# Peilun-Tommy-Li/pHNN-MPC

Hardware: AMD Instinct MI355X
Metric: pHNN-MPC rollouts+grads/sec, cartpole H=50 batch=65536 (higher is better)
Workload: dtype f32

## Files before the change

### phnn_mpc_amd/csrc/phnn_kernels.hip.h

```cpp
#pragma once
#include <hip/hip_runtime.h>

#include <type_traits>

#include "../../include/phnn_mpc.h"
#include "phnn_riccati.hip.h"

#define DEV __device__ __forceinline__
#ifdef PHNN_CACHED_TAPE
#define PHNN_NT_STORE(v, p) (*(p) = (v))
#define PHNN_NT_LOAD(p) (*(p))
#else
#define PHNN_NT_STORE(v, p) __builtin_nontemporal_store((v), (p))
#define PHNN_NT_LOAD(p) __builtin_nontemporal_load((p))
#endif

using f32x4 = __attribute__((ext_vector_type(4))) float;
using f32x2 = __attribute__((ext_vector_type(2))) float;

constexpr int kTileB = 16;
#ifndef PHNN_KMAXWAVES
#define PHNN_KMAXWAVES 8
#endif
constexpr int kMaxWaves = PHNN_KMAXWAVES;
// ... 403 lines not shown
  static constexpr int PART = HID * RS * 2;
  static constexpr int FLOATS = 2 * PART / 4;
};

DEV f16x8 in_frag_h(f32x4 x) {
  f32x2 v01 = {x[0], x[1]}, v23 = {x[2], x[3]};
  f16x2 h01 = __builtin_convertvector(v01, f16x2), h23 = __builtin_convertvector(v23, f16x2);
  f32x2 r01 = residual_h(h01, v01), r23 = residual_h(h23, v23);
  u32x4 B = {__builtin_bit_cast(unsigned, h01), __builtin_bit_cast(unsigned, h23),
             __builtin_bit_cast(unsigned, __builtin_convertvector(r01, f16x2)),
             __builtin_bit_cast(unsigned, __builtin_convertvector(r23, f16x2))};
  return __builtin_bit_cast(f16x8, B);
}
constexpr int kInFragH(int T) { return T * 64 * 4; }
template <int T>
DEV void in_layer_h(Act<T>& o, const float* Wh, Lane ln, f16x8 xf) {
  keep_lds_reads_local();
#pragma unroll
  for (int nt = 0; nt < T; ++nt) o.v[nt] = mfma_h(*reinterpret_cast<const f16x8*>(Wh + (nt * 64 + ln.lane) * 4), xf, o.v[nt]);
}
constexpr int kInHFwd = 1, kInHRecomp = 2, kInHHvp = 4, kInHNet1 = 8, kInHNet1Adj = 16;
#ifndef PHNN_INH_MASK
#define PHNN_INH_MASK (kInHFwd | kInHRecomp | kInHHvp | kInHNet1 | kInHNet1Adj)
#endif
template <int T, int MM, int SITE>
DEV void in_layer_mm(Act<T>& o, const float* Lnet, int oF, int oFh, Lane ln, f32x4 x, int tile0 = 0) {
  if constexpr (MM == MM_F16X2 && (PHNN_INH_MASK & SITE) != 0) in_layer_h<T>(o, Lnet + oFh + tile0 * 256, ln, in_frag_h(x));
  else in_layer<T>(o, Lnet + oF + tile0 * 64, ln, sel4(x, ln.q));
}

DEV void mfma3x2(f32x4& o0, f32x4& o1, const f16x8 (&a)[2][2], f16x8 xh, f16x8 xl) {
  o0 = mfma_h(a[0][1], xh, o0);
  o1 = mfma_h(a[1][1], xh, o1);
  o0 = mfma_h(a[0][0], xl, o0);
  o1 = mfma_h(a[1][0], xl, o1);
  o0 = mfma_h(a[0][0], xh, o0);
  o1 = mfma_h(a[1][0], xh, o1);
}

struct NoEpi {
  DEV void operator()(int, int) const {}
};
#ifndef PHNN_FUSE_SITES
#define PHNN_FUSE_SITES 15
#endif
#ifdef PHNN_NO_FUSED_EPILOGUE
constexpr int kFuseSites = 0;
#else
constexpr int kFuseSites = PHNN_FUSE_SITES;
#endif
constexpr int kFuseK1Act = 1, kFuseK1Red = 2, kFuseK2Act = 4, kFuseK2Red = 8;
#define PHNN_FUSE_K1 (kFuseK1Act | kFuseK1Red)
#define PHNN_FUSE_K2 (kFuseK2Act | kFuseK2Red)
template <int T, class Epi>
DEV void epi_slices(Epi& epi, int P, int s) {
  constexpr int NS = T / 2;
#pragma unroll
  for (int j = (4 * s) / NS; j < (4 * (s + 1)) / NS; ++j) epi(P, j);
}
template <int T, class Epi>
DEV void epi_tail(Epi& epi) {
#pragma unroll
  for (int j = 0; j < 4; ++j) epi(T / 2 - 1, j);
}

template <int T, class Epi = NoEpi>
DEV void sq_fwd_h(Act<T>& o, const float* Wimg, Lane ln, const Split2<T>& in, Epi epi = Epi()) {
  constexpr bool FUSED = !std::is_same_v<Epi, NoEpi>;
  using I = HfImg<16 * T>;
  keep_lds_reads_local();
  matrix_phase_begin();
  const char* base = reinterpret_cast<const char*>(Wimg) + ln.i * (I::RS * 2) + ln.q * 16;
#ifndef PHNN_NO_PREFETCH_FRAGS
  {
    constexpr int PD = 1, NB = PD + 1;
    f16x8 a[NB][2][2];
    auto loadg = [&](int g, f16x8 (&dst)[2][2]) {
      const int n0 = 2 * (g / (T / 2)), s = g % (T / 2);
#pragma unroll
      for (int gg = 0; gg < 2; ++gg)
#pragma unroll
        for (int p = 0; p < 2; ++p)
          dst[gg][p] = *reinterpret_cast<const f16x8*>(base + p * I::PART + (n0 + gg) * 16 * (I::RS * 2) + s * 64);
    };
    constexpr int NG = (T / 2) * (T / 2);
#pragma unroll
    for (int g = 0; g < PD && g < NG; ++g) loadg(g, a[g % NB]);
#pragma unroll
    for (int g = 0; g < NG; ++g) {
      if (g + PD < NG) loadg(g + PD, a[(g + PD) % NB]);
      __builtin_amdgcn_sched_barrier(0);
      const int n0 = 2 * (g / (T / 2)), s = g % (T / 2);
      mfma3x2(o.v[n0], o.v[n0 + 1], a[g % NB], in.h[s], in.l[s]);
      if constexpr (FUSED)
        if (n0 > 0) epi_slices<T>(epi, n0 / 2 - 1, s);
      __builtin_amdgcn_sched_barrier(0);
    }
    matrix_phase_end();
    if constexpr (FUSED) epi_tail<T>(epi);
    return;
  }
#endif
#pragma unroll
  for (int n0 = 0; n0 < T; n0 += 2) {
    if constexpr (FUSED)
      if (n0 > 0) {
// ... 323 lines not shown
    a = z > 0.f ? z : expm1f(z);
    d1 = z > 0.f ? 1.0f : __builtin_amdgcn_exp2f(z * 1.4426950408889634f);
  } else if (ACT == ACT_GELU) {
    const float c = gelu_cdf(z);
    a = z * c;
    d1 = __builtin_fmaf(z, gelu_pdf(z), c);
  } else {
    const float s = __builtin_amdgcn_rcpf(1.0f + __builtin_amdgcn_exp2f(z * -1.4426950408889634f));
    a = z * s;
    d1 = __builtin_fmaf(a, 1.0f - s, s);
  }
}
template <int ACT>
DEV float act_d2(float z) {
  if (ACT == ACT_RELU) return 0.0f;
  if (ACT == ACT_ELU) return z > 0.f ? 0.0f : __builtin_amdgcn_exp2f(z * 1.4426950408889634f);
  if (ACT == ACT_GELU) return gelu_pdf(z) * fmaxf(__builtin_fmaf(-z, z, 2.0f), -3.0e38f);
  const float s = __builtin_amdgcn_rcpf(1.0f + __builtin_amdgcn_exp2f(z * -1.4426950408889634f));
  return s * (1.0f - s) * __builtin_fmaf(z, 1.0f - 2.0f * s, 2.0f);
}
template <int ACT, int T>
DEV void act_of(const Act<T>& z, Act<T>& a) {
#pragma unroll
  for (int t = 0; t < T; ++t)
#pragma unroll
    for (int r = 0; r < 4; ++r) {
      float av, d;
      act_eval<ACT>(z.v[t][r], av, d);
      a.v[t][r] = av;
    }
}
template <int ACT, int T>
DEV void mul_d1(Act<T>& g, const Act<T>& z) {
#pragma unroll
  for (int t = 0; t < T; ++t)
#pragma unroll
    for (int r = 0; r < 4; ++r) {
      float a, d;
      act_eval<ACT>(z.v[t][r], a, d);
      g.v[t][r] *= d;
    }
}

constexpr int TAPE_NONE = 0, TAPE_MPC = 1, TAPE_TRAIN = 2;
template <class M, int TK>
constexpr int tape_floats() {
  if constexpr (TK == TAPE_MPC && M::CURV) return M::TAPE_C;
  else return M::STASH;
}

template <int HID>
struct HTape {
  Act<HID / 16> a1, a2, q1;
};

template <int HID, bool WANT_H, int ACT>
DEV f32x4 hnet_grad_g(const float* L, Lane ln, f32x4 x, HTape<HID>& tp, float& Hval) {
  using Y = LayH2<HID, MM_F32>;
  constexpr int T = Y::T;
  load_vec<T>(tp.a1, L + Y::oB1, ln);
  in_layer<T>(tp.a1, L + Y::oW1f, ln, sel4(x, ln.q));
  {
    Act<T> a;
    act_of<ACT, T>(tp.a1, a);
    load_vec<T>(tp.a2, L + Y::oB2, ln);
    sq_fwd<T, T>(tp.a2, L + Y::oW2, ln, a);
  }
  Act<T> g;
  float s = 0.f;
  keep_lds_reads_local();
#pragma unroll
  for (int t = 0; t < T; ++t) {
    f32x4 w3 = *reinterpret_cast<const f32x4*>(L + Y::oW3 + 16 * t + 4 * ln.q);
#pragma unroll
    for (int r = 0; r < 4; ++r) {
      float a, d;
      act_eval<ACT>(tp.a2.v[t][r], a, d);
      if (WANT_H) s = __builtin_fmaf(w3[r], a, s);
      g.v[t][r] = w3[r] * d;
    }
  }
  if (WANT_H) Hval = reduce_q(s) + L[Y::oB3];
  zero_act<T>(tp.q1);
  sq_bwd<T, T>(tp.q1, L + Y::oW2, ln, g);
#pragma unroll
  for (int t = 0; t < T; ++t) g.v[t] = tp.q1.v[t];
  mul_d1<ACT, T>(g, tp.a1);
  return to4_rep<T>(L + Y::oW1T, ln, g);
}
template <int HID, int ACT>
DEV void hnet_layer1_g(const float* L, Lane ln, f32x4 x, Act<HID / 16>& z1) {
  using Y = LayH2<HID, MM_F32>;
  load_vec<Y::T>(z1, L + Y::oB1, ln);
  in_layer<Y::T>(z1, L + Y::oW1f, ln, sel4(x, ln.q));
}
template <int HID, int ACT>
DEV f32x4 hnet_hvp_g(const float* L, Lane ln, HTape<HID>& tp, f32x4 v) {
  using Y = LayH2<HID, MM_F32>;
  constexpr int T = Y::T;
  Act<T> ad1, w;
  zero_act<T>(ad1);
  in_layer<T>(ad1, L + Y::oW1f, ln, sel4(v, ln.q));
#pragma unroll
  for (int t = 0; t < T; ++t)
#pragma unroll
    for (int r = 0; r < 4; ++r) {
      const float z = tp.a1.v[t][r], zd = ad1.v[t][r];
// ... 58 lines not shown
        if (e == 2 && t + 1 < T) {
          if (WANT_H) w3 = *reinterpret_cast<const f32x4*>(L + Y::oW3 + 16 * (t + 1) + 4 * ln.q);
          w3b = *reinterpret_cast<const f32x4*>(L + Y::oW3B + 16 * (t + 1) + 4 * ln.q);
        }
        split_put_h<T>(spg, P, j, g);
      };
    };
    if (kPreScaled<T> && c == 1.0f) sq_fwd_h<T>(tp.a2, L + Y::oW2, ln, sp, act(std::true_type()));
    else sq_fwd_h<T>(tp.a2, L + Y::oW2, ln, sp, act(std::false_type()));
  } else if (MM == MM_BF16X3) {
    Split3<T> sp;
    split_act<T>(tp.a1, sp);
    sq_fwd_bf<T>(tp.a2, L + Y::oW2, ln, sp);
  } else if (MM == MM_F16X2) {
    Split2<T> sp;
    split_act_h<T>(tp.a1, sp);
    sq_fwd_h<T>(tp.a2, L + Y::oW2, ln, sp);
  } else {
    sq_fwd<T, T>(tp.a2, L + Y::oW2, ln, tp.a1);
  }
  if constexpr (FUSE_ACT) {
  } else if (MM == MM_F16X2 || kPreScaled<T>) {
    const float c = L[Y::oB3 + 1];
    if (kPreScaled<T> && c == 1.0f) {
      tanh_act_pre<T>(tp.a2);
    } else {
#pragma unroll
      for (int t = 0; t < T; ++t)
#pragma unroll
        for (int r = 0; r < 4; ++r) tp.a2.v[t][r] = tanh_scaled(tp.a2.v[t][r], c);
    }
  } else {
    tanh_act<T>(tp.a2);
  }
  Act<T> g;
  keep_lds_reads_local();
  if constexpr (!FUSE_ACT) {
#pragma unroll
    for (int t = 0; t < T; ++t) {
      if (WANT_H) {
        f32x4 w3 = *reinterpret_cast<const f32x4*>(L + Y::oW3 + 16 * t + 4 * ln.q);
#pragma unroll
        for (int r = 0; r < 4; ++r) s = __builtin_fmaf(w3[r], tp.a2.v[t][r], s);
      }
      f32x4 w3b = *reinterpret_cast<const f32x4*>(L + Y::oW3B + 16 * t + 4 * ln.q);
      g.v[t] = w3b * dtanh(tp.a2.v[t]);
    }
  }
  if (WANT_H) Hval = reduce_q(s) + L[Y::oB3];
  zero_act<T>(tp.q1);
  if constexpr (FUSABLE) {
    if constexpr (!FUSE_ACT) split_act_h<T>(g, spg);
    if constexpr (FUSE_RED) {
      To4Pairs<T> red(L + Y::oW1T, ln);
      sq_bwd_h<T>(tp.q1, L + Y::oW2, ln, spg, [&](int P, int j) {
        const int t = 2 * P + (j >> 1), e = 2 * (j & 1);
        const float a0 = tp.a1.v[t][e], a1 = tp.a1.v[t][e + 1];
        red.put(P, j, tp.q1.v[t][e] * __builtin_fmaf(-a0, a0, 1.0f), tp.q1.v[t][e + 1] * __builtin_fmaf(-a1, a1, 1.0f));
      });
      return red.finish();
    } else {
      sq_bwd_h<T>(tp.q1, L + Y::oW2, ln, spg);
    }
  } else if (MM == MM_BF16X3) {
    Split3<T> sp;
    split_act<T>(g, sp);
    sq_bwd_bf<T>(tp.q1, L + Y::oW2, ln, sp);
  } else if (MM == MM_F16X2) {
    Split2<T> sp;
    split_act_h<T>(g, sp);
    sq_bwd_h<T>(tp.q1, L + Y::oW2, ln, sp);
  } else {
    sq_bwd<T, T>(tp.q1, L + Y::oW2, ln, g);
  }
#pragma unroll
  for (int t = 0; t < T; ++t) g.v[t] = tp.q1.v[t] * dtanh(tp.a1.v[t]);
  return to4_rep<T>(L + Y::oW1T, ln, g);
}

template <int HID, int MM, int ACT = ACT_TANH>
DEV void hnet_layer1(const float* L, Lane ln, f32x4 z, Act<HID / 16>& a1) {
  if constexpr (ACT != ACT_TANH) return hnet_layer1_g<HID, ACT>(L, ln, z, a1);
  using Y = LayH2<HID, MM>;
  load_vec<Y::T>(a1, L + Y::oB1, ln);
  in_layer_mm<Y::T, MM, kInHRecomp>(a1, L, Y::oW1f, Y::oW1h, ln, z);
  tanh_act_pre<Y::T>(a1);
}

template <int HID>
struct CurvImg {
  static constexpr int RS = HID + 16, PART = 10 * RS * 2;
  static constexpr int oConst = 2 * PART / 4;
  static constexpr int FLOATS = oConst + 4;
};
struct Curv {
  float m[16];
};
template <int T>
DEV void hnet_curv_operand(const Act<T>& q1, const Act<T>& a1, Split2<T>& sp) {
  Act<T> c;
#pragma unroll
  for (int t = 0; t < T; ++t) c.v[t] = (q1.v[t] * dtanh(a1.v[t])) * a1.v[t];
  split_act_h<T>(c, sp);
}
template <int HID>
DEV f32x4 hnet_curv_kstep(const float* P, Lane ln, int s, f16x8 ch, f16x8 cl) {
  using I = CurvImg<HID>;
  keep_lds_reads_local();
  const int a = ln.i >> 2, b = ln.i & 3, lo = a < b ? a : b, hi = a < b ? b : a;
  const int row = (lo * (9 - lo)) / 2 + (hi - lo);
  const char* base = reinterpret_cast<const char*>(P) + row * (I::RS * 2) + ln.q * 16 + s * 64;
  const f16x8 ah = *reinterpret_cast<const f16x8*>(base);
  const f16x8 al = *reinterpret_cast<const f16x8*>(base + I::PART);
  return mfma_h(ah, ch, mfma_h(ah, cl, mfma_h(al, ch, splat4(0.f))));
}
template <int HID>
DEV f32x4 hnet_curv(const float* P, Lane ln, const HTape<HID>& tp) {
  constexpr int T = HID / 16;
  Split2<T> sp;
  hnet_curv_operand<T>(tp.q1, tp.a1, sp);
  f32x4 tot = hnet_curv_kstep<HID>(P, ln, 0, sp.h[0], sp.l[0]);
#pragma unroll
  for (int s = 1; s < T / 2; ++s) tot = tot + hnet_curv_kstep<HID>(P, ln, s, sp.h[s], sp.l[s]);
  return tot * P[CurvImg<HID>::oConst];
}
DEV void spread_curv(f32x4 mine, Lane ln, Curv& c) {
#pragma unroll
  for (int r = 0; r < 4; ++r)
#pragma unroll
    for (int j = 0; j < 4; ++j) c.m[4 * r + j] = __shfl(mine[j], 16 * r + ln.i);
}
DEV f32x4 curv_apply(const Curv& c, f32x4 v) {
  f32x4 o;
#pragma unroll
  for (int r = 0; r < 4; ++r) {
    float s = 0.f;
#pragma unroll
    for (int j = 0; j < 4; ++j) s = __builtin_fmaf(c.m[4 * r + j], v[j], s);
    o[r] = s;
  }
  return o;
}

template <int HID, bool COMPACT>
DEV void hnet_tape_store(float* stash, int oC, const float* P, Lane ln, const HTape<HID>& tp, f32x4 dH) {
  constexpr int T = HID / 16;
  store_act<T>(stash, ln, tp.a2);
  if constexpr (COMPACT) {
    if (ln.q == 0) PHNN_NT_STORE(dH, reinterpret_cast<f32x4*>(stash + T * 256) + ln.i);
    PHNN_NT_STORE(hnet_curv<HID>(P, ln, tp), reinterpret_cast<f32x4*>(stash + oC) + ln.i * 4 + ln.q);
  } else {
    store_act<T>(stash + T * 256, ln, tp.q1);
    if (ln.q == 0) PHNN_NT_STORE(dH, reinterpret_cast<f32x4*>(stash + 2 * T * 256) + ln.i);
  }
}
template <int T, bool COMPACT>
DEV f32x4 tape_load_dH(const float* stash, Lane ln) {
  return PHNN_NT_LOAD(reinterpret_cast<const f32x4*>(stash + (COMPACT ? 1 : 2) * T * 256) + ln.i);
}
DEV void load_curv(const float* src, Lane ln, Curv& c) {
  const f32x4* p = reinterpret_cast<const f32x4*>(src) + ln.i * 4;
#pragma unroll
  for (int k = 0; k < 4; ++k) {
    f32x4 v = PHNN_NT_LOAD(p + k);
#pragma unroll
    for (int e = 0; e < 4; ++e) c.m[4 * k + e] = v[e];
  }
}
template <int HID, bool COMPACT>
DEV void hnet_tape_load(const float* stash, int oC, Lane ln, HTape<HID>& tp, Curv& cv) {
  constexpr int T = HID / 16;
  load_act<T>(stash, ln, tp.a2);
  if constexpr (COMPACT) load_curv(stash + oC, ln, cv);
  else load_act<T>(stash + T * 256, ln, tp.q1);
}

DEV int pow2_exponent(float mx) {
  int e = 0;
  (void)__builtin_frexpf(mx, &e);
  return (mx > 0.f && mx < 3.0e38f) ? e : 0;
}
DEV f32x4 pow2_normalise(f32x4 v, float& unscale) {
  float mx = fmaxf(fmaxf(__builtin_fabsf(v[0]), __builtin_fabsf(v[1])), fmaxf(__builtin_fabsf(v[2]), __builtin_fabsf(v[3])));
  const int e = pow2_exponent(mx);
  v = v * __builtin_ldexpf(1.0f, -e);
  unscale = __builtin_ldexpf(1.0f, e);
  return v;
}

template <int HID, int MM = MM_F32, bool WG = false, int ACT = ACT_TANH, int SITE = kInHHvp, bool CQ = false, int FE = 0>
DEV f32x4 hnet_hvp(const float* L, Lane ln, HTape<HID>& tp, f32x4 v, float* rec = nullptr, const Curv* cv = nullptr) {
  static_assert(!CQ || (MM == MM_F16X2 && ACT == ACT_TANH && !WG), "the curvature block exists for f16x2 Tanh MPC kernels");
  if constexpr (ACT != ACT_TANH) {
    static_assert(!WG, "weight-gradient kernels exist for Tanh models only");
    return hnet_hvp_g<HID, ACT>(L, ln, tp, v);
  }
  using Y = LayH2<HID, MM>;
  constexpr int T = Y::T;
  float unscale = 1.0f;
  if (MM == MM_F16X2) v = pow2_normalise(v, unscale);
  Act<T> ad1, w;
  zero_act<T>(ad1);
  in_layer_mm<T, MM, SITE>(ad1, L, Y::oW1f, Y::oW1h, ln, v);
#pragma unroll
  for (int t = 0; t < T; ++t) ad1.v[t] = dtanh(tp.a1.v[t]) * ad1.v[t];
  if constexpr (!CQ) {
#pragma unroll
    for (int t = 0; t < T; ++t) tp.q1.v[t] = tp.q1.v[t] * (tp.a1.v[t] * ad1.v[t]);
  }
  zero_act<T>(w);
  constexpr bool FUSABLE = CQ && T >= 2 && T % 2 == 0;
  constexpr bool FUSE_ACT = FUSABLE && (FE & kFuseSites & kFuseK2Act) != 0, FUSE_RED = FUSABLE && (FE & kFuseSites & kFuseK2Red) != 0;
  Split2<T> spw{};
  if constexpr (FUSE_ACT) {
    Split2<T> sp;
    split_act_h<T>(ad1, sp);
    f32x4 w3 = *reinterpret_cast<const f32x4*>(L + Y::oW3S + 4 * ln.q);
    sq_fwd_h<T>(w, L + Y::oW2, ln, sp, [&](int P, int j) {
      const int t = 2 * P + (j >> 1), e = 2 * (j & 1);
      f32x2 x;
#pragma unroll
      for (int k = 0; k < 2; ++k) {
        const float a2 = tp.a2.v[t][e + k];
        const float ad2 = __builtin_fmaf(-a2, a2, 1.0f) * w.v[t][e + k];
        x[k] = w3[e + k] * (a2 * ad2);
      }
      if (e == 2 && t + 1 < T) w3 = *reinterpret_cast<const f32x4*>(L + Y::oW3S + 16 * (t + 1) + 4 * ln.q);
      split_put_h<T>(spw, P, j, x);
    });
  } else {
    if (MM == MM_BF16X3) {
      Split3<T> sp;
      split_act<T>(ad1, sp);
      sq_fwd_bf<T>(w, L + Y::oW2, ln, sp);
    } else if (MM == MM_F16X2) {
      Split2<T> sp;
      split_act_h<T>(ad1, sp);
      sq_fwd_h<T>(w, L + Y::oW2, ln, sp);
    } else {
      sq_fwd<T, T>(w, L + Y::oW2, ln, ad1);
    }
    keep_lds_reads_local();
#pragma unroll
    for (int t = 0; t < T; ++t) {
      f32x4 w3 = *reinterpret_cast<const f32x4*>(L + Y::oW3S + 16 * t + 4 * ln.q);
      f32x4 a2 = tp.a2.v[t];
      f32x4 ad2 = dtanh(a2) * w.v[t];
      if (WG) PHNN_REC_STORE(ad2 * unscale, reinterpret_cast<f32x4*>(rec + 2 * T * 256) + t * 64 + ln.lane);
      w.v[t] = w3 * (a2 * ad2);
    }
  }
  Act<T> qd;
  zero_act<T>(qd);
  if constexpr (FUSABLE) {
    if constexpr (!FUSE_ACT) split_act_h<T>(w, spw);
    if constexpr (FUSE_RED) {
      To4Pairs<T> red(L + Y::oW1T, ln);
      sq_bwd_h<T>(qd, L + Y::oW2, ln, spw, [&](int P, int j) {
        const int t = 2 * P + (j >> 1), e = 2 * (j & 1);
        const float a0 = tp.a1.v[t][e], a1 = tp.a1.v[t][e + 1];
        red.put(P, j, qd.v[t][e] * __builtin_fmaf(-a0, a0, 1.0f), qd.v[t][e + 1] * __builtin_fmaf(-a1, a1, 1.0f));
      });
      return (red.finish() * (-2.0f * L[Y::oB3 + 2]) + curv_apply(*cv, v)) * unscale;
    } else {
      sq_bwd_h<T>(qd, L + Y::oW2, ln, spw);
    }
  } else if (MM == MM_BF16X3) {
    Split3<T> sp;
    split_act<T>(w, sp);
    sq_bwd_bf<T>(qd, L + Y::oW2, ln, sp);
  } else if (MM == MM_F16X2) {
    Split2<T> sp;
    split_act_h<T>(w, sp);
    sq_bwd_h<T>(qd, L + Y::oW2, ln, sp);
  } else {
    sq_bwd<T, T>(qd, L + Y::oW2, ln, w);
  }
  if (WG) store_rec_scaled<T>(rec + 3 * T * 256, ln, qd, unscale);
#pragma unroll
  for (int t = 0; t < T; ++t) {
    if constexpr (CQ) qd.v[t] = qd.v[t] * dtanh(tp.a1.v[t]);
    else qd.v[t] = __builtin_elementwise_fma(qd.v[t], dtanh(tp.a1.v[t]), tp.q1.v[t]);
  }
  f32x4 Hv = to4_rep<T>(L + Y::oW1T, ln, qd);
  if constexpr (CQ) return (Hv * (-2.0f * L[Y::oB3 + 2]) + curv_apply(*cv, v)) * unscale;
  return Hv * (-2.0f * unscale * L[Y::oB3 + 2]);
}

template <int HID, int MM>
DEV f32x4 h1_out_hf(const float* L, Lane ln, const Split2<HID / 16>& sp) {
  using Y = LayH1<HID, MM>;
  constexpr int T = Y::T;
  keep_lds_reads_local();
  const char* base = reinterpret_cast<const char*>(L + Y::oV2) + ln.i * (Y::RS * 2) + ln.q * 16;
  f32x4 o0 = splat4(0.f), o1 = splat4(0.f), o2 = splat4(0.f);
#pragma unroll
  for (int s = 0; s < T / 2; ++s) {
    f16x8 ah = *reinterpret_cast<const f16x8*>(base + s * 64);
    f16x8 al = *reinterpret_cast<const f16x8*>(base + Y::FPART + s * 64);
    o0 = mfma_h(al, sp.h[s], o0);
    o1 = mfma_h(ah, sp.l[s], o1);
    o2 = mfma_h(ah, sp.h[s], o2);
  }
  const float inv = L[Y::oSc];
  f32x4 c2 = *reinterpret_cast<const f32x4*>(L + Y::oC2 + 4 * ln.q);
  return ((o0 + o1) + o2) * inv + c2;
}

template <int HID, int MM>
DEV void h1_bwd_operands(const float* L, Lane ln, const float (&obar)[16], f16x8& b1, f16x8& b2, float& unscale) {
  using Y = LayH1<HID, MM>;
  float mx = 0.f;
#pragma unroll
  for (int k = 0; k < 16; ++k) mx = fmaxf(mx, __builtin_fabsf(obar[k]));
// ... 113 lines not shown
template <int N>
DEV void sym_from_rf(const float (&rf)[16], float (&S)[N][N]) {
#pragma unroll
  for (int i = 0; i < N; ++i) {
    S[i][i] = rf[i * N + i];
#pragma unroll
    for (int j = i + 1; j < N; ++j) S[i][j] = S[j][i] = (rf[i * N + j] + rf[j * N + i]) * 0.5f;
  }
}
template <int N>
DEV void rbar_from(f32x4 lam, f32x4 dH, const float (&Stl)[N], const float (&StdH)[N], float (&rbar)[16]) {
  float m[N][N];
#pragma unroll
  for (int k = 0; k < 16; ++k) rbar[k] = 0.f;
#pragma unroll
  for (int i = 0; i < N; ++i)
#pragma unroll
    for (int j = 0; j < N; ++j) m[i][j] = __builtin_fmaf(lam[i], StdH[j], dH[i] * Stl[j]);
#pragma unroll
  for (int i = 0; i < N; ++i) {
    rbar[i * N + i] = -m[i][i];
#pragma unroll
    for (int j = i + 1; j < N; ++j) rbar[i * N + j] = rbar[j * N + i] = (m[i][j] + m[j][i]) * -0.5f;
  }
}

template <int N_, int HID_, bool FIXG_, int MM_ = MM_F32, int MI_ = 1, int ACT_ = ACT_TANH>
struct PhnnModel {
  static constexpr int N = N_, HID = HID_, T = HID / 16, MM = MM_, MI = MI_, ACT = ACT_;
  static constexpr bool FIXG = FIXG_, SPLIT = false;
  static_assert(N_ * MI_ <= 16 && MI_ <= 4, "G_net output n*m <= 16, m <= 4");
  static constexpr int SCR = kScrFloats;
  static constexpr int oH = 0;
  static constexpr int oR = oH + LayH2<HID, MM>::SIZE;
  static constexpr int oGn = oR + LayH1<HID, MM>::SIZE;
  static constexpr int oJ = oGn + (FIXG ? 0 : LayH1<HID, MM>::SIZE);
  static constexpr int oG = oJ + 16;
  static constexpr int oP = oG + 16;
  static constexpr bool CURV = MM == MM_F16X2 && ACT == ACT_TANH &&
                               sizeof(float) * (oP + CurvImg<HID>::FLOATS + kMaxWaves * SCR) <= kMaxLdsBytes;
  static constexpr int IMG = oP + (CURV ? CurvImg<HID>::FLOATS : 0);
  static constexpr int FUSE = (HID_ != 128 || !FIXG_) ? 0 : ((MI_ <= 2 ? PHNN_FUSE_K1 : 0) | (MI_ == 1 ? PHNN_FUSE_K2 : 0));

  static constexpr int oStashRf = 2 * T * 256 + 64;
  static constexpr int STASH = oStashRf + 256;
  static constexpr int oTapeRf = T * 256 + 64, oTapeC = oTapeRf + 256, TAPE_C = oTapeC + 256;

  template <bool WANT_H, int TK = TAPE_NONE, int FE = 0>
  DEV static f32x4 f(const float* L, float* scr, Lane ln, f32x4 x, f32x4 u, float& Hval, float* stash = nullptr) {
    constexpr bool ST = TK != TAPE_NONE, CT = TK == TAPE_MPC && CURV;
    keep_lds_reads_local();
    HTape<HID> tp;
    f32x4 dH = hnet_grad<HID, WANT_H, MM, kInHFwd, ACT, FE>(L + oH, ln, x, tp, Hval);
    if (ST) hnet_tape_store<HID, CT>(stash, oTapeC, L + oP, ln, tp, dH);
    Act<T> hR;
    float rf[16];
    h1_fwd<HID, MM, kInHNet1, ACT>(L + oR, scr, ln, x, hR, rf, ST ? stash + (CT ? oTapeRf : oStashRf) : nullptr);
    float G[N * MI];
    if (FIXG) {
#pragma unroll
      for (int i = 0; i < N * MI; ++i) G[i] = L[oG + i];
    } else {
      Act<T> hG;
      float gf[16];
      h1_fwd<HID, MM, kInHNet1, ACT>(L + oGn, scr, ln, x, hG, gf);
#pragma unroll
      for (int i = 0; i < N * MI; ++i) G[i] = gf[i];
    }
    return combine(L, rf, dH, G, u);
  }

  DEV static f32x4 combine(const float* L, const float (&rf)[16], f32x4 dH, const float (&G)[N * MI], f32x4 u) {
    float S[N][N], StdH[N];
    sym_from_rf<N>(rf, S);
#pragma unroll
    for (int k = 0; k < N; ++k) {
      float a = 0.f;
#pragma unroll
      for (int i = 0; i < N; ++i) a = __builtin_fmaf(S[i][k], dH[i], a);
      StdH[k] = a;
    }
    f32x4 dx = splat4(0.f);
#pragma unroll
    for (int i = 0; i < N; ++i) {
      float acc = 0.f;
#pragma unroll
      for (int j = 0; j < N; ++j) acc = __builtin_fmaf(L[oJ + i * N + j], dH[j], acc);
#pragma unroll
      for (int k = 0; k < N; ++k) acc = __builtin_fmaf(-S[i][k], StdH[k], acc);
      if (MI == 1) {
        dx[i] = __builtin_fmaf(G[i], u[0], acc);
      } else {
        float gu = 0.f;
#pragma unroll
        for (int k = 0; k < MI; ++k) gu = __builtin_fmaf(G[i * MI + k], u[k], gu);
        dx[i] = acc + gu;
      }
    }
    return dx;
  }

  static constexpr bool RECHB = !LayH1<HID, MM>::HF;
  static constexpr int NBIG = 4 + (RECHB ? (FIXG ? 1 : 2) : 0);
  using Rec = WRec<T, NBIG>;

  static constexpr bool UBAR_DIRECT = FIXG;
  DEV static f32x4 ubar_direct(const float* L, f32x4 lam) {
// ... 203 lines not shown
      mnet_fwd(L + oMn, ln, f32x4{y[0], y[1], 0.f, 0.f}, mt);
      mass_from_outputs<MT>(mt.o, m, w);
    }
  }

  DEV static float Base_Gu(const float* L, int row, f32x4 u) {
    float s = 0.f;
#pragma unroll
    for (int k = 0; k < MI; ++k) s = __builtin_fmaf(L[oCG + row * MI + k], u[k], s);
    return s;
  }
  DEV static f32x4 Base_Gt(const float* L, float dpb0, float dpb1) {
    f32x4 ub = splat4(0.f);
#pragma unroll
    for (int k = 0; k < MI; ++k) ub[k] = L[oCG + 2 * MI + k] * dpb0 + L[oCG + 3 * MI + k] * dpb1;
    return ub;
  }

  static constexpr int STASH = 2 * T * 256 + 64;
  static constexpr int oTapeC = T * 256 + 64, TAPE_C = oTapeC + 256;

  struct CartZ { float a, b, c, sn, bc; f32x4 z; };
  DEV static CartZ cart_z(const float* L, f32x4 y) {
    CartZ r;
    r.a = L[oC + 0], r.b = L[oC + 1], r.c = L[oC + 2];
    float cs;
    sincos_dev(y[1], r.sn, cs);
    r.bc = r.b * cs;
    r.z = f32x4{y[0], y[1], r.a * y[2] + r.bc * y[3], r.bc * y[2] + r.c * y[3]};
    return r;
  }
  DEV static f32x4 cart_f_tail(const float* L, const CartZ& cz, f32x4 dH, f32x4 u) {
    const float a = cz.a, c = cz.c, bc = cz.bc;
    const f32x4 z = cz.z;
    float dp0 = (-dH[0] - L[oC + 6] * dH[2]) + Base_Gu(L, 2, u);
    float dp1 = (-dH[1] - L[oC + 7] * dH[3]) + Base_Gu(L, 3, u);
    float det = (a * c - bc * bc) + 1e-6f;
    float mi00 = c / det, mi01 = -bc / det, mi11 = a / det;
    return f32x4{mi00 * z[2] + mi01 * z[3], mi01 * z[2] + mi11 * z[3], mi00 * dp0 + mi01 * dp1,
                 mi01 * dp0 + mi11 * dp1};
  }

  template <bool WANT_H, int TK = TAPE_NONE, int FE = 0>
  DEV static f32x4 f(const float* L, float* scr, Lane ln, f32x4 y, f32x4 u, float& Hval, float* stash = nullptr) {
    constexpr bool ST = TK != TAPE_NONE, CT = TK == TAPE_MPC && CURV;
    keep_lds_reads_local();
    if constexpr (MT != MASS_CARTPOLE) {
      float m[3], w[3];
      MTape mt;
      mass_eval(L, ln, y, m, w, mt);
      f32x4 z = {y[0], y[1], m[0] * y[2] + m[1] * y[3], m[1] * y[2] + m[2] * y[3]};
      HTape<HID> tp;
      f32x4 dH = hnet_grad<HID, WANT_H, MM, kInHFwd, ACT, FE>(L + oH, ln, z, tp, Hval);
      if (ST) hnet_tape_store<HID, CT>(stash, oTapeC, L + oP, ln, tp, dH);
      float dp0 = (-dH[0] - L[oC + 6] * dH[2]) + Base_Gu(L, 2, u);
      float dp1 = (-dH[1] - L[oC + 7] * dH[3]) + Base_Gu(L, 3, u);
      return f32x4{w[0] * z[2] + w[1] * z[3], w[1] * z[2] + w[2] * z[3], w[0] * dp0 + w[1] * dp1, w[1] * dp0 + w[2] * dp1};
    }
    const CartZ cz = cart_z(L, y);
    HTape<HID> tp;
    f32x4 dH = hnet_grad<HID, WANT_H, MM, kInHFwd, ACT, FE>(L + oH, ln, cz.z, tp, Hval);
    if (ST) hnet_tape_store<HID, CT>(stash, oTapeC, L + oP, ln, tp, dH);
    return cart_f_tail(L, cz, dH, u);
  }

  static constexpr int NBIG = 4;
  using Rec = WRec<T, NBIG>;

  template <bool ST = false, bool WG = false, int INH = -1, int FE = 0>
  DEV static void vjp(const float* L, float* scr, Lane ln, f32x4 y, f32x4 u, f32x4 lam, f32x4& ybar, f32x4& ubar,
                      const float* stash = nullptr, float* rec = nullptr, float Hbar = 0.f) {
    constexpr bool CQ = CURV && !WG;
    Curv cv;
    keep_lds_reads_local();
    if constexpr (MT != MASS_CARTPOLE) {
      float m[3], w[3];
      MTape mt;
      mass_eval(L, ln, y, m, w, mt);
      f32x4 z = {y[0], y[1], m[0] * y[2] + m[1] * y[3], m[1] * y[2] + m[2] * y[3]};
      HTape<HID> tp;
      float Hdummy;
      f32x4 dH;
      if (ST) {
        dH = tape_load_dH<T, CQ>(stash, ln);
        hnet_tape_load<HID, CQ>(stash, oTapeC, ln, tp, cv);
        hnet_layer1<HID, MM, ACT>(L + oH, ln, z, tp.a1);
      } else {
        dH = hnet_grad<HID, false, MM, INH & kInHRecomp, ACT>(L + oH, ln, z, tp, Hdummy);
        if constexpr (CQ) spread_curv(hnet_curv<HID>(L + oP, ln, tp), ln, cv);
      }
      const float Rd2 = L[oC + 6], Rd3 = L[oC + 7];
      const float dp0 = (-dH[0] - Rd2 * dH[2]) + Base_Gu(L, 2, u);
      const float dp1 = (-dH[1] - Rd3 * dH[3]) + Base_Gu(L, 3, u);
      const float pb0 = lam[0] * w[0] + lam[1] * w[1], pb1 = lam[0] * w[1] + lam[1] * w[2];
      const float dpb0 = lam[2] * w[0] + lam[3] * w[1], dpb1 = lam[2] * w[1] + lam[3] * w[2];
      f32x4 v = {-dpb0, -dpb1, -Rd2 * dpb0, -Rd3 * dpb1};
      ubar = Base_Gt(L, dpb0, dpb1);
      if (WG) {
        if (!ST) {
          store_rec<T>(rec, ln, tp.a2);
          store_rec<T>(rec + Rec::VEC, ln, tp.q1);
        }
        if (ln.q == 0) {
          f32x4* sm = reinterpret_cast<f32x4*>(rec + Rec::oSmall + ln.i * kRecSmall);
          sm[0] = z;
          sm[1] = v;
          sm[2] = lam;
          sm[3] = dH;
          sm[4] = f32x4{0.f, 0.f, -dpb0 * dH[2], -dpb1 * dH[3]};
          sm[8] = u;
          sm[9] = f32x4{Hbar, 0.f, 0.f, 0.f};
        }
      }
      f32x4 zb = hnet_hvp<HID, MM, WG, ACT, INH & kInHHvp, CQ, ST ? FE : 0>(L + oH, ln, tp, v, rec, &cv);
      if (WG) zb = zb + Hbar * dH;
// ... 721 lines not shown
  if (c.has_x_min) {
    no_speculation();
#pragma unroll
    for (int i = 0; i < N; ++i) g[i] = __builtin_fmaf(-2.0f * c.barrier_weight, fmaxf(c.x_min[i] - x[i], 0.f), g[i]);
  }
  if (c.has_x_max) {
    no_speculation();
#pragma unroll
    for (int i = 0; i < N; ++i) g[i] = __builtin_fmaf(2.0f * c.barrier_weight, fmaxf(x[i] - c.x_max[i], 0.f), g[i]);
  }
  return g;
}

struct RollParams {
  const float* img;
  const float* x0;
  const float* u;
  const float* traj_in;
  const float* traj_bar;
  const float* cost_bar;
  float* cost;
  float* traj;
  float* grad_u;
  float* grad_x0;
  float* stash;
  const float* dx_bar;
  float* dx_out;
  float* wrec;
  int no_cost;
  long long B;
  int H;
  float dt, half_dt, sixth_dt;
  phnn_cost c;
  float Qs[16];
  const float* x_ref;
  long long ref_bs, ref_ts;
  int ref_rows;
  const int* ref_off_dev;
  int ref_off_host;
};

struct PointParams {
  const float* img;
  const float* x;
  const float* u;
  const float* lam;
  float* dx;
  float* Hout;
  long long B;
  const float* Hbar;
  float* wrec;
};

template <int IMG>
DEV void stage_image(float* lds, const float* img) {
  const f32x4* src = reinterpret_cast<const f32x4*>(img);
  f32x4* dst = reinterpret_cast<f32x4*>(lds);
  for (int k = threadIdx.x; k < IMG / 4; k += blockDim.x) dst[k] = src[k];
  __syncthreads();
}

template <int N>
DEV f32x4 load_state(const float* p) {
  if (N == 4) return *reinterpret_cast<const f32x4*>(p);
  f32x4 x = splat4(0.f);
#pragma unroll
  for (int i = 0; i < N; ++i) x[i] = p[i];
  return x;
}
template <int N>
DEV void store_state(float* p, f32x4 x) {
  if (N == 4) {
    *reinterpret_cast<f32x4*>(p) = x;
  } else {
#pragma unroll
    for (int i = 0; i < N; ++i) p[i] = x[i];
  }
}

DEV float clamp_u(const phnn_cost& c, float u, bool on = true) {
  const bool b = on && c.has_u_bounds;
  const float lo = b ? c.u_min : -INFINITY, hi = b ? c.u_max : INFINITY;
  const float r = fminf(fmaxf(u, lo), hi);
  return u == u ? r : u;
}
DEV float clamp_u_k1(const phnn_cost& c, float u) { return c.has_u_bounds && u == u ? fminf(fmaxf(u, c.u_min), c.u_max) : u; }

template <int MI>
DEV f32x4 load_u(const float* up, int t) {
  f32x4 u = splat4(0.f);
#pragma unroll
  for (int k = 0; k < MI; ++k) u[k] = up[t * MI + k];
  return u;
}
template <int MI>
DEV f32x4 clamp_u4(const phnn_cost& c, f32x4 u, bool on = true) {
#pragma unroll
  for (int k = 0; k < MI; ++k) u[k] = clamp_u(c, u[k], on);
  return u;
}
template <int MI>
DEV float control_cost(const phnn_cost& c, f32x4 u) {
  if (MI == 1) return (u[0] * c.R[0]) * u[0];
  float cost = 0.f;
#pragma unroll
  for (int j = 0; j < MI; ++j) {
    float s = 0.f;
#pragma unroll
    for (int i = 0; i < MI; ++i) s = __builtin_fmaf(u[i], c.R[i * MI + j], s);
    cost = __builtin_fmaf(s, u[j], cost);
  }
// ... 89 lines not shown
  constexpr int N = M::N;
  constexpr bool STASH = TK != TAPE_NONE;
  using SS = StashStep<M, INTEG, STASH ? TK : TAPE_MPC>;
  const Lane ln = tc.ln;
  float* scr = tc.scr;
  const long long tile = tc.tile, b = tc.b;
  const bool writer = tc.writer;
  f32x4 x = load_state<N>(p.x0 + b * N);
  if (p.traj && writer) store_state<N>(p.traj + (b * (p.H + 1)) * N, x);
  RefRows<N> rr;
  float cost;
  if constexpr (REF) {
    rr.init(p, b);
    cost = state_cost<N>(p.c, x, rr.row(0));
  } else {
    cost = state_cost<N>(p.c, x, p.c.x_target);
  }
  constexpr int MI = M::MI;
  const float* up = p.u + b * p.H * MI;
  float Hd;
  for (int t = 0; t < p.H; ++t) {
    f32x4 tgt;
    if constexpr (REF) tgt = rr.row(t + 1);
    f32x4 u = load_u<MI>(up, t);
#pragma unroll
    for (int k = 0; k < MI; ++k) u[k] = clamp_u_k1(p.c, u[k]);
    if (MI == 1) cost = __builtin_fmaf(u[0] * p.c.R[0], u[0], cost);
    else cost += control_cost<MI>(p.c, u);
    float* sl = STASH ? p.stash + (tile * p.H + t) * (long long)SS::FLOATS : nullptr;
    f32x4 k1 = M::template f<false, TK, kFuseEpi<M, INTEG, REF, TK == TAPE_MPC, kFuseK1Act | kFuseK1Red>>(L, scr, ln, x, u, Hd, sl);
    if (p.dx_out && writer) store_state<N>(p.dx_out + (b * p.H + t) * N, k1);
    if (INTEG == PHNN_INTEG_EULER) {
      x = x + p.dt * k1;
    } else {
      constexpr int SLOT = SS::SLOT;
      f32x4 acc = k1, kp = k1;
#pragma unroll 1
      for (int s = 1; s < 4; ++s) {
        const f32x4 y = x + (s == 3 ? p.dt : p.half_dt) * kp;
        float* ss = STASH ? sl + s * SLOT : nullptr;
        if (STASH) store_stage(ss + SS::TAPE, ln, y);
        kp = M::template f<false, TK>(L, scr, ln, y, u, Hd, ss);
        acc = acc + (s == 3 ? 1.0f : 2.0f) * kp;
      }
      x = x + p.sixth_dt * acc;
    }
    if constexpr (REF) cost += state_cost<N>(p.c, x, tgt);
    else cost += state_cost<N>(p.c, x, p.c.x_target);
    if (p.traj && writer) store_state<N>(p.traj + (b * (p.H + 1) + t + 1) * N, x);
  }
  if (writer && p.cost) p.cost[b] = cost;
}

template <class M, int INTEG, int TK, bool REF = false>
__global__ __launch_bounds__(64 * kMaxWaves) void k_rollout_fwd(RollParams p) {
  extern __shared__ __attribute__((aligned(16))) float lds[];
  stage_image<M::IMG>(lds, p.img);
  TileCtx tc;
  if (!tile_ctx<M>(tc, lds, p.B)) return;
  fwd_march<M, INTEG, TK, REF>(p, lds, tc);
}

template <class M, int INTEG, bool STASH, bool WG = false, bool REF = false>
DEV void grad_march(const RollParams& p, const float* L, const TileCtx& tc) {
  constexpr int N = M::N;
  using SS = StashStep<M, INTEG, WG ? TAPE_TRAIN : TAPE_MPC>;
  const Lane ln = tc.ln;
  float* scr = tc.scr;
  const long long tile = tc.tile, b = tc.b;
  const bool valid = tc.valid, writer = tc.writer;
  const float* tr = p.traj_in + (b * (p.H + 1)) * N;
  constexpr int MI = M::MI;
  const float* up = p.u + b * p.H * MI;
  const float cb = p.no_cost ? 0.0f : (p.cost_bar ? p.cost_bar[b] : 1.0f);
  const float* tb = p.traj_bar ? p.traj_bar + (b * (p.H + 1)) * N : nullptr;
  const float* db = p.dx_bar ? p.dx_bar + (b * p.H) * N : nullptr;
  const float live = valid ? 1.0f : 0.0f;
  RefRows<N> rr;
  f32x4 lam;
  if constexpr (REF) {
    rr.init(p, b);
    lam = cb * state_cost_grad<N>(p.c, p.Qs, load_state<N>(tr + (long long)p.H * N), rr.row(p.H));
  } else {
    lam = cb * state_cost_grad<N>(p.c, p.Qs, load_state<N>(tr + (long long)p.H * N), p.c.x_target);
  }
  if (tb) lam = lam + load_state<N>(tb + (long long)p.H * N);
  if (WG) lam = lam * live;
  constexpr int STAGES = INTEG == PHNN_INTEG_EULER ? 1 : 4;
  float Hd;
  for (int t = p.H - 1; t >= 0; --t) {
    f32x4 x = load_state<N>(tr + (long long)t * N);
    f32x4 tgt;
    if constexpr (REF && INTEG == PHNN_INTEG_EULER) tgt = rr.row(t);
    f32x4 uraw = load_u<MI>(up, t);
    f32x4 u = clamp_u4<MI>(p.c, uraw, !p.no_cost);
    f32x4 dxb = splat4(0.f);
    if (INTEG == PHNN_INTEG_EULER && db) dxb = load_state<N>(db + (long long)t * N) * live;
    f32x4 xb, ub, utot;
    float* rec = nullptr;
    if constexpr (WG) rec = p.wrec + ((tile * p.H + t) * STAGES) * (long long)M::Rec::SIZE;
    if constexpr (INTEG == PHNN_INTEG_EULER) {
      bool skipped = false;
      if constexpr (kStep0Skip<M, INTEG, WG>) {
        if (t == 0 && !p.grad_x0 && !p.traj_bar) {
          utot = M::ubar_direct(L, p.dt * lam + dxb);
          skipped = true;
        }
      }
      if (!skipped) {
        if constexpr (WG) {
// ... 19 lines not shown
          y2 = s == 0 ? y : y2;
          y3 = s == 1 ? y : y3;
          y4 = s == 2 ? y : y4;
        }
      }
      f32x4 ysum = splat4(0.f), ybn = ysum;
      utot = splat4(0.f);
#pragma unroll 1
      for (int s = 3; s >= 0; --s) {
        f32x4 y;
        if constexpr (STASH) y = s == 0 ? load_state<N>(tr + (long long)t * N) : load_stage(sl + s * SLOT + SS::TAPE, ln);
        else y = s == 0 ? load_state<N>(tr + (long long)t * N) : (s == 1 ? y2 : (s == 2 ? y3 : y4));
        const f32x4 us = clamp_u4<MI>(p.c, load_u<MI>(up, t), !p.no_cost);
        f32x4 in = ((s == 0 || s == 3) ? p.sixth_dt : 2.0f * p.sixth_dt) * lam;
        if (s != 3) in = in + (s == 2 ? p.dt : p.half_dt) * ybn;
        if (s == 0 && db) in = in + load_state<N>(db + (long long)t * N) * live;
        f32x4 yb;
        if constexpr (WG) M::template vjp<STASH, true>(L, scr, ln, y, us, in, yb, ub, STASH ? sl + s * SLOT : nullptr, rec + s * M::Rec::SIZE);
        else M::template vjp<STASH>(L, scr, ln, y, us, in, yb, ub, STASH ? sl + s * SLOT : nullptr);
        utot = s == 3 ? ub : utot + ub;
        ybn = yb;
        ysum = s == 3 ? yb : ysum + yb;
      }
      lam = lam + ysum;
      x = load_state<N>(tr + (long long)t * N);
      if constexpr (REF) tgt = rr.row(t);
      uraw = load_u<MI>(up, t);
      u = clamp_u4<MI>(p.c, uraw, !p.no_cost);
    }
    if constexpr (REF) lam = lam + cb * state_cost_grad<N>(p.c, p.Qs, x, tgt);
    else lam = lam + cb * state_cost_grad<N>(p.c, p.Qs, x, p.c.x_target);
    if (tb) lam = lam + load_state<N>(tb + (long long)t * N) * (WG ? live : 1.0f);
#pragma unroll
    for (int k = 0; k < MI; ++k) {
      float g;
      if (MI == 1) {
        g = __builtin_fmaf(cb * (2.0f * p.c.R[0]), u[0], utot[0]);
      } else {
        float s = 0.f;
#pragma unroll
        for (int j = 0; j < MI; ++j) s = __builtin_fmaf(p.c.R[k * MI + j] + p.c.R[j * MI + k], u[j], s);
        g = __builtin_fmaf(cb, s, utot[k]);
      }
      if (!p.no_cost && p.c.has_u_bounds && !(uraw[k] >= p.c.u_min && uraw[k] <= p.c.u_max)) g = 0.f;
      if (writer && p.grad_u) p.grad_u[(b * p.H + t) * MI + k] = g;
    }
  }
  if (p.grad_x0 && writer) store_state<N>(p.grad_x0 + b * N, lam);
}

template <class M, int INTEG, bool STASH, bool WG = false, bool REF = false>
__global__ __launch_bounds__(64 * kMaxWaves) void k_rollout_grad(RollParams p) {
  extern __shared__ __attribute__((aligned(16))) float lds[];
  stage_image<M::IMG>(lds, p.img);
  TileCtx tc;
  if (!tile_ctx<M>(tc, lds, p.B)) return;
  grad_march<M, INTEG, STASH, WG, REF>(p, lds, tc);
}


template <class M>
__global__ __launch_bounds__(64 * kMaxWaves) void k_model_forward(PointParams p) {
  extern __shared__ __attribute__((aligned(16))) float lds[];
  constexpr int N = M::N;
  stage_image<M::IMG>(lds, p.img);
  const int wave = threadIdx.x >> 6, nwaves = blockDim.x >> 6;
  const Lane ln = make_lane();
  float* scr = lds + M::IMG + wave * M::SCR;
  const long long ntiles = (p.B + kTileB - 1) / kTileB;
  for (long long tile = (long long)blockIdx.x * nwaves + wave; tile < ntiles; tile += (long long)gridDim.x * nwaves) {
    long long b = tile * kTileB + ln.i;
    const bool valid = b < p.B;
    if (!valid) b = p.B - 1;
    f32x4 x = load_state<N>(p.x + b * N);
    float Hval = 0.f;
    f32x4 dx = M::template f<true>(lds, scr, ln, x, load_u<M::MI>(p.u + b * M::MI, 0), Hval);
    if (valid && ln.q == 0) {
      store_state<N>(p.dx + b * N, dx);
      if (p.Hout) p.Hout[b] = Hval;
    }
  }
}

template <class M, bool WG = false>
__global__ __launch_bounds__(64 * kMaxWaves) void k_model_vjp(PointParams p) {
  extern __shared__ __attribute__((aligned(16))) float lds[];
  constexpr int N = M::N;
  stage_image<M::IMG>(lds, p.img);
  const int wave = threadIdx.x >> 6, nwaves = blockDim.x >> 6;
  const Lane ln = make_lane();
  float* scr = lds + M::IMG + wave * M::SCR;
  const long long ntiles = (p.B + kTileB - 1) / kTileB;
  for (long long tile = (long long)blockIdx.x * nwaves + wave; tile < ntiles; tile += (long long)gridDim.x * nwaves) {
    long long b = tile * kTileB + ln.i;
    const bool valid = b < p.B;
    if (!valid) b = p.B - 1;
    f32x4 x = load_state<N>(p.x + b * N);
    f32x4 lam = load_state<N>(p.lam + b * N);
    f32x4 xb, ub;
    const f32x4 u = load_u<M::MI>(p.u + b * M::MI, 0);
    if constexpr (WG) {
      const float live = valid ? 1.0f : 0.0f;
      M::template vjp<false, true>(lds, scr, ln, x, u, lam * live, xb, ub, nullptr,
                                   p.wrec + tile * (long long)M::Rec::SIZE, p.Hbar ? p.Hbar[b] * live : 0.0f);
    } else {
      M::template vjp<false, false, 0>(lds, scr, ln, x, u, lam, xb, ub);
    }
// ... 741 lines not shown
```

Baseline: 33.08 million.

## Fuse curvature operand into backward epilogue, compute dtanh once, burst-stage LDS image

Builds the split f16 curvature operand inside the fused backward-reduction epilogue and keeps it in the tape struct, so hnet_curv no longer recomputes q1*dtanh(a1)*a1 afterwards. In the HVP path, dtanh(a1) is computed once and overwrites a1, so the later reduction epilogue reuses it instead of recomputing 1-a^2. The weight-image staging into LDS now issues batches of 8/4/2/1 loads per thread before the stores, to raise memory-level parallelism. In exchange the tape carries extra Split2 registers, which may raise register pressure and lower occupancy.

```diff
diff --git a/phnn_mpc_amd/csrc/phnn_kernels.hip.h b/phnn_mpc_amd/csrc/phnn_kernels.hip.h
--- a/phnn_mpc_amd/csrc/phnn_kernels.hip.h
+++ b/phnn_mpc_amd/csrc/phnn_kernels.hip.h
@@ -479,6 +479,17 @@
 constexpr int kFuseK1Act = 1, kFuseK1Red = 2, kFuseK2Act = 4, kFuseK2Red = 8;
 #define PHNN_FUSE_K1 (kFuseK1Act | kFuseK1Red)
 #define PHNN_FUSE_K2 (kFuseK2Act | kFuseK2Red)
+constexpr int kCurvFromQ1 = 0, kCurvFragments = 2;
+#ifdef PHNN_NO_EPI_CURV
+constexpr int kCurvFused = kCurvFromQ1;
+#else
+constexpr int kCurvFused = kCurvFragments;
+#endif
+#ifdef PHNN_NO_D1_ONCE
+constexpr bool kD1Once = false;
+#else
+constexpr bool kD1Once = true;
+#endif
 template <int T, class Epi>
 DEV void epi_slices(Epi& epi, int P, int s) {
   constexpr int NS = T / 2;
@@ -908,7 +919,11 @@
 template <int HID>
 struct HTape {
   Act<HID / 16> a1, a2, q1;
-};
+  Split2<HID / 16> cs;
+};
+template <int HID, int MM, int ACT, int FE>
+constexpr int kCurvForm = (MM == MM_F16X2 && ACT == ACT_TANH && HID >= 32 && HID % 32 == 0 && (FE & kFuseSites & kFuseK1Red) != 0)
+                              ? kCurvFused : kCurvFromQ1;
 
 template <int HID, bool WANT_H, int ACT>
 DEV f32x4 hnet_grad_g(const float* L, Lane ln, f32x4 x, HTape<HID>& tp, float& Hval) {
@@ -1073,11 +1088,15 @@
   if constexpr (FUSABLE) {
     if constexpr (!FUSE_ACT) split_act_h<T>(g, spg);
     if constexpr (FUSE_RED) {
+      constexpr int CF = kCurvForm<HID, MM, ACT, FE>;
+      if constexpr (CF == kCurvFragments) tp.cs = Split2<T>{};
       To4Pairs<T> red(L + Y::oW1T, ln);
       sq_bwd_h<T>(tp.q1, L + Y::oW2, ln, spg, [&](int P, int j) {
         const int t = 2 * P + (j >> 1), e = 2 * (j & 1);
         const float a0 = tp.a1.v[t][e], a1 = tp.a1.v[t][e + 1];
-        red.put(P, j, tp.q1.v[t][e] * __builtin_fmaf(-a0, a0, 1.0f), tp.q1.v[t][e + 1] * __builtin_fmaf(-a1, a1, 1.0f));
+        const float g0 = tp.q1.v[t][e] * __builtin_fmaf(-a0, a0, 1.0f), g1 = tp.q1.v[t][e + 1] * __builtin_fmaf(-a1, a1, 1.0f);
+        if constexpr (CF == kCurvFragments) split_put_h<T>(tp.cs, P, j, f32x2{g0 * a0, g1 * a1});
+        red.put(P, j, g0, g1);
       });
       return red.finish();
     } else {
@@ -1135,11 +1154,12 @@
   const f16x8 al = *reinterpret_cast<const f16x8*>(base + I::PART);
   return mfma_h(ah, ch, mfma_h(ah, cl, mfma_h(al, ch, splat4(0.f))));
 }
-template <int HID>
+template <int HID, int CF = kCurvFromQ1>
 DEV f32x4 hnet_curv(const float* P, Lane ln, const HTape<HID>& tp) {
   constexpr int T = HID / 16;
   Split2<T> sp;
-  hnet_curv_operand<T>(tp.q1, tp.a1, sp);
+  if constexpr (CF == kCurvFragments) sp = tp.cs;
+  else hnet_curv_operand<T>(tp.q1, tp.a1, sp);
   f32x4 tot = hnet_curv_kstep<HID>(P, ln, 0, sp.h[0], sp.l[0]);
 #pragma unroll
   for (int s = 1; s < T / 2; ++s) tot = tot + hnet_curv_kstep<HID>(P, ln, s, sp.h[s], sp.l[s]);
@@ -1163,13 +1183,14 @@
   return o;
 }
 
-template <int HID, bool COMPACT>
+template <int HID, bool COMPACT, int CF = kCurvFromQ1>
 DEV void hnet_tape_store(float* stash, int oC, const float* P, Lane ln, const HTape<HID>& tp, f32x4 dH) {
+  static_assert(COMPACT || CF == kCurvFromQ1, "the training tape stores q1 itself");
   constexpr int T = HID / 16;
   store_act<T>(stash, ln, tp.a2);
   if constexpr (COMPACT) {
     if (ln.q == 0) PHNN_NT_STORE(dH, reinterpret_cast<f32x4*>(stash + T * 256) + ln.i);
-    PHNN_NT_STORE(hnet_curv<HID>(P, ln, tp), reinterpret_cast<f32x4*>(stash + oC) + ln.i * 4 + ln.q);
+    PHNN_NT_STORE((hnet_curv<HID, CF>(P, ln, tp)), reinterpret_cast<f32x4*>(stash + oC) + ln.i * 4 + ln.q);
   } else {
     store_act<T>(stash + T * 256, ln, tp.q1);
     if (ln.q == 0) PHNN_NT_STORE(dH, reinterpret_cast<f32x4*>(stash + 2 * T * 256) + ln.i);
@@ -1223,15 +1244,23 @@
   Act<T> ad1, w;
   zero_act<T>(ad1);
   in_layer_mm<T, MM, SITE>(ad1, L, Y::oW1f, Y::oW1h, ln, v);
-#pragma unroll
-  for (int t = 0; t < T; ++t) ad1.v[t] = dtanh(tp.a1.v[t]) * ad1.v[t];
-  if constexpr (!CQ) {
-#pragma unroll
-    for (int t = 0; t < T; ++t) tp.q1.v[t] = tp.q1.v[t] * (tp.a1.v[t] * ad1.v[t]);
-  }
-  zero_act<T>(w);
   constexpr bool FUSABLE = CQ && T >= 2 && T % 2 == 0;
   constexpr bool FUSE_ACT = FUSABLE && (FE & kFuseSites & kFuseK2Act) != 0, FUSE_RED = FUSABLE && (FE & kFuseSites & kFuseK2Red) != 0;
+  constexpr bool D1 = kD1Once && FUSE_RED;
+#pragma unroll
+  for (int t = 0; t < T; ++t) {
+    if constexpr (D1) {
+      tp.a1.v[t] = dtanh(tp.a1.v[t]);
+      ad1.v[t] = tp.a1.v[t] * ad1.v[t];
+    } else {
+      ad1.v[t] = dtanh(tp.a1.v[t]) * ad1.v[t];
+    }
+  }
+  if constexpr (!CQ) {
+#pragma unroll
+    for (int t = 0; t < T; ++t) tp.q1.v[t] = tp.q1.v[t] * (tp.a1.v[t] * ad1.v[t]);
+  }
+  zero_act<T>(w);
   Split2<T> spw{};
   if constexpr (FUSE_ACT) {
     Split2<T> sp;
@@ -1280,7 +1309,8 @@
       sq_bwd_h<T>(qd, L + Y::oW2, ln, spw, [&](int P, int j) {
         const int t = 2 * P + (j >> 1), e = 2 * (j & 1);
         const float a0 = tp.a1.v[t][e], a1 = tp.a1.v[t][e + 1];
-        red.put(P, j, qd.v[t][e] * __builtin_fmaf(-a0, a0, 1.0f), qd.v[t][e + 1] * __builtin_fmaf(-a1, a1, 1.0f));
+        if constexpr (D1) red.put(P, j, qd.v[t][e] * a0, qd.v[t][e + 1] * a1);
+        else red.put(P, j, qd.v[t][e] * __builtin_fmaf(-a0, a0, 1.0f), qd.v[t][e + 1] * __builtin_fmaf(-a1, a1, 1.0f));
       });
       return (red.finish() * (-2.0f * L[Y::oB3 + 2]) + curv_apply(*cv, v)) * unscale;
     } else {
@@ -1500,7 +1530,7 @@
     keep_lds_reads_local();
     HTape<HID> tp;
     f32x4 dH = hnet_grad<HID, WANT_H, MM, kInHFwd, ACT, FE>(L + oH, ln, x, tp, Hval);
-    if (ST) hnet_tape_store<HID, CT>(stash, oTapeC, L + oP, ln, tp, dH);
+    if (ST) hnet_tape_store<HID, CT, kCurvForm<HID, MM, ACT, FE>>(stash, oTapeC, L + oP, ln, tp, dH);
     Act<T> hR;
     float rf[16];
     h1_fwd<HID, MM, kInHNet1, ACT>(L + oR, scr, ln, x, hR, rf, ST ? stash + (CT ? oTapeRf : oStashRf) : nullptr);
@@ -1810,7 +1840,7 @@
       f32x4 z = {y[0], y[1], m[0] * y[2] + m[1] * y[3], m[1] * y[2] + m[2] * y[3]};
       HTape<HID> tp;
       f32x4 dH = hnet_grad<HID, WANT_H, MM, kInHFwd, ACT, FE>(L + oH, ln, z, tp, Hval);
-      if (ST) hnet_tape_store<HID, CT>(stash, oTapeC, L + oP, ln, tp, dH);
+      if (ST) hnet_tape_store<HID, CT, kCurvForm<HID, MM, ACT, FE>>(stash, oTapeC, L + oP, ln, tp, dH);
       float dp0 = (-dH[0] - L[oC + 6] * dH[2]) + Base_Gu(L, 2, u);
       float dp1 = (-dH[1] - L[oC + 7] * dH[3]) + Base_Gu(L, 3, u);
       return f32x4{w[0] * z[2] + w[1] * z[3], w[1] * z[2] + w[2] * z[3], w[0] * dp0 + w[1] * dp1, w[1] * dp0 + w[2] * dp1};
@@ -1818,7 +1848,7 @@
     const CartZ cz = cart_z(L, y);
     HTape<HID> tp;
     f32x4 dH = hnet_grad<HID, WANT_H, MM, kInHFwd, ACT, FE>(L + oH, ln, cz.z, tp, Hval);
-    if (ST) hnet_tape_store<HID, CT>(stash, oTapeC, L + oP, ln, tp, dH);
+    if (ST) hnet_tape_store<HID, CT, kCurvForm<HID, MM, ACT, FE>>(stash, oTapeC, L + oP, ln, tp, dH);
     return cart_f_tail(L, cz, dH, u);
   }
 
@@ -2646,11 +2676,30 @@
   float* wrec;
 };
 
-template <int IMG>
+template <int NB>
+DEV void stage_burst(f32x4* dst, const f32x4* src, int& k, int n4) {
+  const int nt = blockDim.x;
+  for (; k + (NB - 1) * nt < n4; k += NB * nt) {
+    f32x4 v[NB];
+#pragma unroll
+    for (int i = 0; i < NB; ++i) v[i] = src[k + i * nt];
+#pragma unroll
+    for (int i = 0; i < NB; ++i) dst[k + i * nt] = v[i];
+  }
+}
+template <int IMG, bool BURST = false>
 DEV void stage_image(float* lds, const float* img) {
   const f32x4* src = reinterpret_cast<const f32x4*>(img);
   f32x4* dst = reinterpret_cast<f32x4*>(lds);
-  for (int k = threadIdx.x; k < IMG / 4; k += blockDim.x) dst[k] = src[k];
+  if constexpr (!BURST) {
+    for (int k = threadIdx.x; k < IMG / 4; k += blockDim.x) dst[k] = src[k];
+  } else {
+  int k = threadIdx.x;
+  stage_burst<8>(dst, src, k, IMG / 4);
+  stage_burst<4>(dst, src, k, IMG / 4);
+  stage_burst<2>(dst, src, k, IMG / 4);
+  stage_burst<1>(dst, src, k, IMG / 4);
+  }
   __syncthreads();
 }
 
@@ -2846,10 +2895,18 @@
   if (writer && p.cost) p.cost[b] = cost;
 }
 
+#ifdef PHNN_NO_BURST_STAGING
+template <class M, bool WG>
+constexpr bool kBurstStaging = false;
+#else
+template <class M, bool WG>
+constexpr bool kBurstStaging = M::MM == MM_F16X2 && !WG;
+#endif
+
 template <class M, int INTEG, int TK, bool REF = false>
 __global__ __launch_bounds__(64 * kMaxWaves) void k_rollout_fwd(RollParams p) {
   extern __shared__ __attribute__((aligned(16))) float lds[];
-  stage_image<M::IMG>(lds, p.img);
+  stage_image<M::IMG, kBurstStaging<M, false>>(lds, p.img);
   TileCtx tc;
   if (!tile_ctx<M>(tc, lds, p.B)) return;
   fwd_march<M, INTEG, TK, REF>(p, lds, tc);
@@ -2975,7 +3032,7 @@
 template <class M, int INTEG, bool STASH, bool WG = false, bool REF = false>
 __global__ __launch_bounds__(64 * kMaxWaves) void k_rollout_grad(RollParams p) {
   extern __shared__ __attribute__((aligned(16))) float lds[];
-  stage_image<M::IMG>(lds, p.img);
+  stage_image<M::IMG, kBurstStaging<M, WG>>(lds, p.img);
   TileCtx tc;
   if (!tile_ctx<M>(tc, lds, p.B)) return;
   grad_march<M, INTEG, STASH, WG, REF>(p, lds, tc);
```

New measurement: 32.86 million. Within noise of the previous version (-0.7%).
